# brucechin/OctopusZK

Hardware: AMD Instinct MI355X
Metric: BN254 G1 VariableBaseMSM Mscalar-mul/s at 2^20 (higher is better)
Workload: dtype u32; 1 GPU; VariableBaseMSM BN254 G1 2^20 random scalars/bases per GPU, bit-exact vs the serial CPU path (BASELINE.json configs[1]); n_per_gpu=1048576, window_bits=16, windows=8, glv=True, prepared_bases=False, msms_in_flight=3, schedule=pipeline3, parallelism=index-range shard x1, RCCL all-gather of 192-B partials + HIP point sum

## Files before the change

### include/ozk.h

```cpp
#ifndef OZK_H
#define OZK_H

#include <stddef.h>
#include <stdint.h>

#ifdef __cplusplus
extern "C" {
#endif

#define OZK_OK 0
#define OZK_E_INVALID -1
#define OZK_E_NO_DEVICE -2
#define OZK_E_NOMEM -3
#define OZK_E_INTERNAL -4

#define OZK_G1 1
#define OZK_G2 2

const char* ozk_last_error(void);
int ozk_version(void);
int ozk_device_count(void);
int ozk_device_cu_count(void);
int ozk_stream_create_cu_range(int32_t first_cu, int32_t n_cus, void** stream);
int ozk_stream_destroy(void* stream);
// ... 32 lines not shown
int ozk_var_msm_stage_bytes(int32_t n, int32_t type, size_t* sorted_bytes, size_t* sort_ws_bytes,
                            size_t* accum_ws_bytes);
int ozk_var_msm_sort_dev(const void* d_bases, int32_t prepared, const void* d_scalars, int32_t n, int32_t type,
                         void* d_sorted, size_t sorted_bytes, void* d_sort_ws, size_t sort_ws_bytes, void* stream);
int ozk_var_msm_accum_dev(const void* d_prepared, int32_t n, int32_t type, void* d_sorted, size_t sorted_bytes,
                          void* d_accum_ws, size_t accum_ws_bytes, void* d_tail, size_t tail_bytes, void* stream,
                          int32_t part);

size_t ozk_var_msm_prepared_bytes(int32_t n, int32_t type);
int ozk_var_msm_prepare_dev(const void* d_bases, int32_t n, int32_t type, void* d_prepared, size_t prepared_size,
                            void* stream);
int ozk_var_msm_prepared_dev(const void* d_prepared, const void* d_scalars, int32_t n, int32_t type, void* d_out,
                             void* d_workspace, size_t workspace_bytes, void* stream);
int ozk_bases_create_host(const uint8_t* bases, int32_t n, int32_t type, int32_t task_id, void** handle);
int ozk_var_msm_bases_host(void* handle, const uint8_t* scalars, int32_t n, uint8_t* out);
int ozk_bases_destroy(void* handle);
int ozk_bases_type(void* handle);

int ozk_order_event_create(void** ev);
int ozk_order_event_destroy(void* ev);


int ozk_points_sum_dev(const void* d_points, int32_t k, int32_t type, void* d_out, void* stream);

int ozk_groth16_combine_dev(const void* d_records, int32_t world, void* d_proof, void* stream);

int ozk_prof_enable(int on);
int ozk_prof_dominant_kernel_ms(double* avg_ms, int* launches);
int ozk_prof_dominant_kernel_stats(double* stats4, int* launches);
int ozk_prof_dominant_kernel_clock_mhz(double* stats4, int* launches);
double ozk_prof_clock_khz(void);
int ozk_var_msm_plan(int32_t n, int32_t* window_bits, int32_t* windows);
int ozk_var_msm_glv(int32_t n);

int ozk_gen_bases_dev(uint64_t seed, int32_t n, int32_t type, void* d_out_wire, void* stream);

int ozk_fixed_batch_msm_host(int32_t outerc, int32_t window_size, int32_t out_len,
                             int32_t inner_len, int32_t n, int32_t scalar_size,
                             const uint8_t* base, const uint8_t* scalars, int32_t bn_type,
                             int32_t task_id, uint8_t* out);
int ozk_fixed_double_batch_msm_host(int32_t outerc1, int32_t window_size1, int32_t outerc2,
                                    int32_t window_size2, int32_t out_len1, int32_t inner_len1,
                                    int32_t out_len2, int32_t inner_len2, int32_t n,
                                    const uint8_t* base_g1, const uint8_t* base_g2,
                                    const uint8_t* scalars, int32_t task_id, uint8_t* out);
int ozk_field_batch_mul_host(const uint8_t* in, int32_t n, int32_t task_id, uint8_t* out);

size_t ozk_fixed_batch_msm_workspace_bytes(int32_t outerc, int32_t window_size, int32_t n,
                                           int32_t bn_type);
int ozk_fixed_batch_msm_dev(int32_t outerc, int32_t window_size, int32_t n, const void* d_base,
                            const void* d_scalars, int32_t bn_type, void* d_out,
                            void* d_workspace, size_t workspace_bytes, void* stream);
int ozk_field_batch_mul_dev(const void* d_in, int32_t n, void* d_out, void* stream);
int ozk_fixed_batch_msm_compact_dev(int32_t outerc, int32_t window_size, int32_t n, const void* d_base,
                                    const void* d_scalars, int32_t bn_type, void* d_out, void* d_workspace,
                                    size_t workspace_bytes, void* stream);
int ozk_fixed_batch_msm_compact_host(int32_t outerc, int32_t window_size, int32_t n, const uint8_t* base,
                                     const uint8_t* scalars, int32_t bn_type, int32_t task_id, uint8_t* out);
int ozk_fixed_batch_msm_base_dev(int32_t outerc, int32_t window_size, int32_t n, const uint8_t* base_host,
                                 const void* d_scalars, int32_t bn_type, void* d_out, int32_t compact,
                                 void* d_workspace, size_t workspace_bytes, void* stream);

int ozk_fft_host(const uint8_t* in, int32_t n, const uint8_t* omega, int32_t task_id,
                 uint8_t* out);
size_t ozk_fft_workspace_bytes(int32_t n);
int ozk_fft_dev(const void* d_in, int32_t n, const uint8_t* omega_host32, void* d_out,
// ... 94 lines not shown
```

### octopuszk_amd/build.py

```python
import os
import shutil
import subprocess
import sys

HERE = os.path.dirname(os.path.abspath(__file__))
CSRC = os.path.join(HERE, "csrc")
ROOT = os.path.dirname(HERE)
LIB = os.path.join(HERE, "libozk_hip.so")

HIP_SOURCES = ["msm_var.hip", "msm_var_g2.hip", "msm_fixed.hip", "fft.hip", "host_ctx.hip", "pairing.hip", "msm_multi.hip",
               "point_codec.hip", "points_scale.hip", "ec_fft.hip"]
HEADERS = ["consts_gen.h", "mad_chain_gen.h", "fp29.cuh", "fq2.cuh", "fq12.cuh", "batch_verify.cuh", "point_codec.cuh", "points_scale.cuh", "ec_fft.cuh", "bace.cuh", "pairing_consts_gen.h", "ec.cuh", "quad.cuh", "curve.cuh", "msm_var.cuh", "msm_var_driver.cuh", "msm_multi.cuh", "glv.cuh", "ozk_common.h", "knobs.h", "host_ctx.h", "pin_cache.h",
           os.path.join("..", "..", "include", "ozk.h")]
HIPCC_FLAGS = ["-std=c++17", "-O3", "--offload-arch=gfx950", "-fPIC", "-fno-gpu-rdc", "-Wno-unused-result",
               "-Wno-pass-failed"]

JNI_LIBS = {
    "libAlgebraMSMVariableBaseMSM.so": "jni_var_msm.c",
    "libAlgebraMSMFixedBaseMSM.so": "jni_fixed_msm.c",
    "libAlgebraFFTAuxiliary.so": "jni_fft.c",
}


def _newer(target, deps):
    if not os.path.exists(target):
        return True
    t = os.path.getmtime(target)
    return any(os.path.exists(d) and os.path.getmtime(d) > t for d in deps)


def hipcc():
    for cand in (shutil.which("hipcc"), "/opt/rocm/bin/hipcc"):
        if cand and os.path.exists(cand):
            return cand
    raise RuntimeError("hipcc not found: the HIP library cannot be built (there is no CPU path)")


def build(force=False, verbose=True):
    srcs = [os.path.join(CSRC, s) for s in HIP_SOURCES if os.path.exists(os.path.join(CSRC, s))]
    deps = srcs + [os.path.join(CSRC, h) for h in HEADERS]
    if force or _newer(LIB, deps):
        defs = []
        if os.path.exists(os.path.join(CSRC, "fq2.cuh")):
            defs.append("-DOZK_WITH_G2")
        objdir = os.path.join(HERE, "_obj")
# ... 38 lines not shown
```

### octopuszk_amd/csrc/knobs.h

```cpp
#pragma once
#include <stdlib.h>
#include <string.h>

#include <atomic>
#include <mutex>

namespace ozk {

constexpr int KNOB_COMPUTED = -0x7fffffff;
constexpr int KNOB_STRING = KNOB_COMPUTED + 1;

#define OZK_KNOBS(X)                                                                                                     \
                                                   \
  X(MSM_GLV, "OZK_MSM_GLV", 1, "0: plain 256-bit windows instead of the GLV split (var MSM up to 2^23 pairs, fixed base)") \
  X(MSM_SIGNED, "OZK_MSM_SIGNED", 1, "0: unsigned window digits in the GLV form")                                        \
  X(MSM_C, "OZK_MSM_C", KNOB_COMPUTED, "window bits, 1..16 (default: the cost model's choice)")                          \
  X(MSM_L1, "OZK_MSM_L1", KNOB_COMPUTED, "sorted entries per level-1 lane (default: from the bucket size; 0 as unset)")   \
  X(MSM_L1_ROUNDS, "OZK_MSM_L1_ROUNDS", 2, "most rounds of resident workgroups level 1 is rounded up to; 0: no rounding") \
  X(MSM_TAIL_MODE, "OZK_MSM_TAIL_MODE", -1, "0 / 1: force the latency / throughput shape of the window sums")            \
  X(MSM_SMALL_SORT, "OZK_MSM_SMALL_SORT", 1, "0: small MSMs take the two-level sort too")                                \
  X(MSM_S_LAT, "OZK_MSM_S_LAT", KNOB_COMPUTED, "buckets per lane in a latency tail's fused first level (default: 8 G1, 4 G2)") \
  X(MSM_FIN_MAX, "OZK_MSM_FIN_MAX", 4, "elements per window left to the final one-wave kernel, 1..16")                   \
                                                                                                    \
  X(HOST_SLICES, "OZK_HOST_SLICES", 8, "most slices a host-buffer MSM is cut into; 1: no slicing")                       \
  X(HOST_SLICE_MIN_LOG, "OZK_HOST_SLICE_MIN_LOG", 18, "log2 of the smallest slice")                                      \
  X(SHARD, "OZK_SHARD", 0, "1: the JNI entries shard large calls over the visible devices")                              \
  X(SHARD_MIN_N, "OZK_SHARD_MIN_N", 1 << 21, "smallest call OZK_SHARD=1 shards")                                         \
  X(SHARD_COUNT, "OZK_SHARD_COUNT", 0, "shards of such a call; 0: one per device")                                       \
  X(SHARD_RCCL, "OZK_SHARD_RCCL", 1, "0: the partials of a sharded call go through the host, not RCCL")                  \
  X(COPY_HELPERS, "OZK_COPY_HELPERS", 3, "threads staging host buffers beside the caller, 0..11 (first use only)")       \
  X(HOST_TRACE, "OZK_HOST_TRACE", 0, "1: per-call host timings on stderr; 2: with absolute timestamps")                  \
                                                                                     \
  X(FB_WS, "OZK_FB_WS", KNOB_COMPUTED, "window bits of a GLV fixed-base table (default: cost model, at most the caller's)") \
  X(FB_AFFINE, "OZK_FB_AFFINE", 1, "0: Jacobian gather-add instead of affine table records")                             \
  X(FB_TABLE_CACHE, "OZK_FB_TABLE_CACHE", 1, "0: window tables are built per call")                                      \
  X(FB_TABLE_CACHE_MB, "OZK_FB_TABLE_CACHE_MB", 1024, "MiB of cached window tables per device")                          \
  X(FB_TABLE_CACHE_SECOND_USE, "OZK_FB_TABLE_CACHE_SECOND_USE", 1, "0: a table is cached on its first use")              \
  X(FB_HOST_RANGES, "OZK_FB_HOST_RANGES", 4, "ranges a host fixed-base call downloads its results in")                   \
  X(MM_WS, "OZK_MM_WS", KNOB_COMPUTED, "window bits of the shared-base batched MSM (default: from n)")                   \
                                                                                             \
  X(FFT_MAXK, "OZK_FFT_MAXK", 8, "most butterfly stages per pass, 3..10")                                                \
  X(FFT_PLAN, "OZK_FFT_PLAN", 1, "0: stages spread evenly over the passes")                                              \
  X(FFT_KS, "OZK_FFT_KS", KNOB_STRING, "explicit stages per pass, e.g. \"8,6,8\" (must sum to log2 n)")                  \
  X(FFT_TW_PYRAMID, "OZK_FFT_TW_PYRAMID", 1, "0: twiddles from the flat table")                                          \
  X(FFT_PLAN_CACHE, "OZK_FFT_PLAN_CACHE", 1, "0: twiddle tables are built per call")                                     \
  X(FFT_PLAN_CACHE_MB, "OZK_FFT_PLAN_CACHE_MB", 4096, "MiB of cached twiddle tables per device")                         \
  X(QAP_FOLD_SCALE, "OZK_QAP_FOLD_SCALE", 1, "0: the witness map scales in a pass of its own")                           \
  X(BACE_LDS_SLOTS, "OZK_BACE_LDS_SLOTS", 16, "circuit slots kept in LDS, 0..28")

enum Knob {
// ... 58 lines not shown
```

### octopuszk_amd/csrc/msm_var.cuh

```cuda
#pragma once
#include "curve.cuh"
#include "glv.cuh"

namespace ozk {

constexpr u32 BID_NONE = 0xffffffffu;

struct MsmPlan {
  int n_in;
  int glv;
  int n;
  int sd;
  int c;
  int cb;
  int W;
  int L1;
  int LK;
  int S;
  int lone;
  int small_sort;
  int S_lat;
  int fin_max;
  int tail_mode;
};

OZK_HD u32 scalar_digit(const u32 (&s)[8], int w, int c) {
  const int bit = w * c;
  const int wi = bit >> 5, sh = bit & 31;
  u32 v = s[wi] >> sh;
  if (sh + c > 32 && wi + 1 < 8) v |= s[wi + 1] << (32 - sh);
  return v & ((1u << c) - 1u);
}

OZK_HD bool digit_decode(u32 code, int sd, u32& b, u32& neg) {
  if (sd) {
    const u32 t = code - 1u;
    b = t >> 1;
    neg = t & 1u;
  } else {
    b = code;
    neg = 0;
  }
  return code != 0;
}
template <class Emit>
OZK_HD void signed_digit_codes(const u32 (&e)[8], int c, int W, bool neg, Emit emit) {
  const u32 half = 1u << (c - 1);
  const u32 thr = (c == 16 && neg) ? half - 1u : half;
  u32 cy = 0;
  for (int w = 0; w < W; w++) {
    const u32 d = scalar_digit(e, w, c) + cy;
    cy = d > thr;
    const u32 m = cy ? (1u << c) - d : d;
    emit(w, (uint16_t)(m ? (((m - 1u) << 1) | (cy ^ (u32)neg)) + 1u : 0u));
  }
}
// ... 907 lines not shown
        acc.accumulate(pts_in, idx_in, p);
      }
    }
    }
    if (cur != BID_NONE) {
      if (cur_cb) {
        head_bid = cur;
        acc.store(pts_out + (size_t)(2 * (size_t)t) * IO::REC_WORDS);
        if (cf) {
          tail_bid = cur;
          if constexpr (FIRST) {
            acc.store_infinity(pts_out + (size_t)(2 * (size_t)t + 1) * IO::REC_WORDS);
          } else {
            IO::store_rec_jac(jac_infinity<CV>(), pts_out + (size_t)(2 * (size_t)t + 1) * IO::REC_WORDS);
          }
        }
      } else if (cf) {
        tail_bid = cur;
        acc.store(pts_out + (size_t)(2 * (size_t)t + 1) * IO::REC_WORDS);
      } else {
        acc.store(buckets + (size_t)cur * IO::REC_WORDS);
      }
    }
  }
  bid_out[2 * (size_t)t] = head_bid;
  bid_out[2 * (size_t)t + 1] = tail_bid;
}

template <class CV, bool FIRST, bool LAZY = false>
__global__ void __launch_bounds__(256, (FIRST && CV::LDS_ACC) ? 2 : 1)
k_segreduce(const u32* __restrict__ bid_in, const u32* __restrict__ idx_in, const u32* __restrict__ pts_in,
            const u32* __restrict__ d_count, int n_in_static, int L,
            u32* __restrict__ buckets, u32* __restrict__ bid_out, u32* __restrict__ pts_out,
            int n_lanes, unsigned long long* __restrict__ clk) {
  const int t = blockIdx.x * blockDim.x + threadIdx.x;
  unsigned long long w0 = 0, c0 = 0;
  if constexpr (FIRST) {
    if (clk != nullptr && threadIdx.x == 0) {
      w0 = (unsigned long long)wall_clock64();
      c0 = (unsigned long long)clock64();
      atomicMax(&clk[0], ~w0);
    }
  }
  if (t < n_lanes)
    segreduce_lane<CV, FIRST, LAZY>(t, bid_in, idx_in, pts_in, d_count, n_in_static, L, buckets, bid_out, pts_out);
  if constexpr (FIRST) {
    if (clk != nullptr && (threadIdx.x & 63) == 0) {
      const unsigned long long w1 = (unsigned long long)wall_clock64();
      atomicMax(&clk[1], w1);
      if (threadIdx.x == 0) {
        atomicAdd(&clk[2], (unsigned long long)clock64() - c0);
        atomicAdd(&clk[3], w1 - w0);
      }
    }
  }
}

static __global__ void k_read_clock(unsigned long long* out) { out[0] = (unsigned long long)wall_clock64(); }

template <class CV>
__global__ void __launch_bounds__(256)
k_segreduce_small(const u32* __restrict__ d_count, int n_in, int L, u32* __restrict__ buckets,
                  u32* __restrict__ bid_a, u32* __restrict__ pts_a, u32* __restrict__ bid_b, u32* __restrict__ pts_b) {
  if (*d_count == 0) return;
  u32 *bi = bid_a, *pi = pts_a, *bo = bid_b, *po = pts_b;
  while (true) {
    const int lanes = (n_in + L - 1) / L;
    for (int t = threadIdx.x; t < lanes; t += blockDim.x)
      segreduce_lane<CV, false>(t, bi, nullptr, pi, d_count, n_in, L, buckets, bo, po);
    if (lanes == 1) break;
    block_sync();
    n_in = 2 * lanes;
    u32* tb = bi; bi = bo; bo = tb;
    u32* tp = pi; pi = po; po = tp;
  }
}

constexpr int RUN_MAX = 16;
constexpr int RUNMERGE_BLOCK = 256;
template <class CV>
__global__ void __launch_bounds__(RUNMERGE_BLOCK)
k_runmerge(const u32* __restrict__ bid_in, const u32* __restrict__ pts, int n_slots,
           u32* __restrict__ buckets, u32* __restrict__ bid_out, u32* __restrict__ remaining,
           const u32* __restrict__ hist_src, u32* __restrict__ hist_dst, size_t n_hist) {
  using IO = CurveIO<CV>;
  constexpr bool LIST = !CV::LDS_ACC;
  constexpr int ROUNDS = RUN_MAX / 2;
  constexpr int CAP = 2 * RUNMERGE_BLOCK;
  __shared__ u32 item_s[2][CAP];
  __shared__ uint8_t item_span[2][CAP];
  __shared__ u32 item_cnt[ROUNDS + 1];
  if (threadIdx.x <= ROUNDS) item_cnt[threadIdx.x] = 0;
  const int t = blockIdx.x * blockDim.x + threadIdx.x;
  for (size_t i = (size_t)t; i < n_hist; i += (size_t)gridDim.x * blockDim.x) hist_dst[i] = hist_src[i];
  block_sync();
  u32 alive = 0;
#pragma unroll 1
  for (int k = 0; k < 2; k++) {
    const int x = 2 * t + 1 + k;
    if (x >= n_slots) break;
    const u32 bx = bid_in[x];
    u32 out = BID_NONE;
    if (bx != BID_NONE) {
      int s = x, e = x;
      while (s > 0 && x - s < RUN_MAX && bid_in[s - 1] == bx) s--;
      while (e + 1 < n_slots && e - x < RUN_MAX && bid_in[e + 1] == bx) e++;
      const bool is_short = (x - s < RUN_MAX) && (e - x < RUN_MAX) && (e - s + 1 <= RUN_MAX);
      if (!is_short) {
        out = bx;
      } else if (s == x) {
        if constexpr (!LIST) {
          Xyzz<CV> acc = IO::load_xyzz(pts + (size_t)s * IO::REC_WORDS);
          for (int q = s + 1; q <= e; q += 2) acc = xyzz_add(acc, IO::load_xyzz(pts + (size_t)q * IO::REC_WORDS));
          IO::store_rec_xyzz(acc, buckets + (size_t)bx * IO::REC_WORDS);
        } else if (e > s) {
          const u32 j = atomicAdd(&item_cnt[0], 1u);
          item_s[0][j] = (u32)s;
          item_span[0][j] = (uint8_t)(e - s);
        } else {
          IO::store_rec_xyzz(IO::load_xyzz(pts + (size_t)s * IO::REC_WORDS), buckets + (size_t)bx * IO::REC_WORDS);
        }
      }
    }
    bid_out[x] = out;
    alive += (out != BID_NONE);
  }
  if (t == 0 && n_slots > 0) {
    bid_out[0] = bid_in[0];
    alive += (bid_in[0] != BID_NONE);
  }
  for (int o = 32; o > 0; o >>= 1) alive += __shfl_xor(alive, o);
  if ((threadIdx.x & 63) == 0 && alive) atomicAdd(remaining, alive);
#pragma unroll 1
  for (int r = 0; LIST && r < ROUNDS; r++) {
    block_sync();
    const u32 len = (u32)__builtin_amdgcn_readfirstlane((int)item_cnt[r]);
    if (len == 0) break;
    const int cur = r & 1;
#pragma unroll 1
    for (u32 i = threadIdx.x; i < len; i += RUNMERGE_BLOCK) {
      const u32 s = item_s[cur][i];
      const u32 span = item_span[cur][i];
      u32* bucket = buckets + (size_t)bid_in[s] * IO::REC_WORDS;
      const u32 off = 2u * (u32)r + 1u;
      const u32* sum = r == 0 ? pts + (size_t)s * IO::REC_WORDS : bucket;
      const Xyzz<CV> acc = xyzz_add(IO::load_xyzz(sum), IO::load_xyzz(pts + ((size_t)s + off) * IO::REC_WORDS));
      IO::store_rec_xyzz(acc, bucket);
      if (off + 2u <= span) {
        const u32 j = atomicAdd(&item_cnt[r + 1], 1u);
        item_s[cur ^ 1][j] = s;
        item_span[cur ^ 1][j] = (uint8_t)span;
      }
    }
  }
}

template <class CV, bool FIRSTLEVEL>
__global__ void __launch_bounds__(256)
k_wsum(const u32* __restrict__ A_in, const u32* __restrict__ R_in, const u32* __restrict__ hist,
       int m_in, int S, int g, u32* __restrict__ A_out, u32* __restrict__ R_out, int m_out, int W, int prio) {
  using IO = CurveIO<CV>;
  if (prio) __builtin_amdgcn_s_setprio(3);
  const int t = blockIdx.x * blockDim.x + threadIdx.x;
  if (t >= m_out * W) return;
  const int w = t / m_out, j = t - w * m_out;
  const size_t base = (size_t)w * m_in;
  const int lo = j * S;
  int hi = lo + S;
  if (hi > m_in) hi = m_in;
  Jac<CV> run = jac_infinity<CV>(), ws = jac_infinity<CV>(), asum = jac_infinity<CV>();
  for (int e = hi - 1; e >= lo; e--) {
    if constexpr (FIRSTLEVEL) {
      if (hist[base + e] != 0) run = jac_add(run, IO::load_rec(R_in + (base + e) * IO::REC_WORDS));
    } else {
      run = jac_add(run, IO::load_jac(R_in + (base + e) * IO::JAC_WORDS));
    }
    if (e > lo) ws = jac_add(ws, run);
    if constexpr (!FIRSTLEVEL) asum = jac_add(asum, IO::load_jac(A_in + (base + e) * IO::JAC_WORDS));
  }
  for (int k = 0; k < g; k++) ws = jac_dbl(ws);
  if constexpr (!FIRSTLEVEL) ws = jac_add(ws, asum);
  IO::store_jac(ws, A_out + ((size_t)w * m_out + j) * IO::JAC_WORDS);
  IO::store_jac(run, R_out + ((size_t)w * m_out + j) * IO::JAC_WORDS);
}

// ... 254 lines not shown
```

### octopuszk_amd/csrc/msm_var.hip

```cpp
#include "msm_var_driver.cuh"

#include <dlfcn.h>
#include <rccl/rccl.h>

#include <algorithm>
#include <chrono>
#include <new>
#include <string>
#include <thread>
#include <vector>

OZK_G2_DRIVER_INSTANCES(extern)

using namespace ozk;

template <class F>
static auto with_plan(int n, int type, F f) {
  return by_point_type(type, [&](auto t) { return f(t, plan_for<typename decltype(t)::CV>(n, false)); });
}
#define CV_OF(t) typename decltype(t)::CV

extern "C" {

size_t ozk_var_msm_workspace_bytes(int32_t n, int32_t type) {
// ... 732 lines not shown
  OZK_HIP(hipDeviceSynchronize());
  std::vector<unsigned long long> h((size_t)g_prof.count * 4);
  if (g_prof.count) OZK_HIP(hipMemcpy(h.data(), g_prof.d_clk, h.size() * sizeof(unsigned long long), hipMemcpyDeviceToHost));
  std::vector<double> m;
  double tot = 0;
  for (int i = 0; i < g_prof.count; i++) {
    if (h[4 * i + 3] == 0) continue;
    const double mhz = (double)h[4 * i + 2] / (double)h[4 * i + 3] * g_prof.clk_khz * 1e-3;
    m.push_back(mhz);
    tot += mhz;
  }
  *launches = (int)m.size();
  if (m.empty()) return OZK_OK;
  std::sort(m.begin(), m.end());
  stats4[0] = tot / (double)m.size();
  stats4[1] = m[m.size() / 2];
  stats4[2] = m.front();
  stats4[3] = m.back();
  return OZK_OK;
}

double ozk_prof_clock_khz(void) { return g_prof.clk_khz; }

int ozk_var_msm_plan(int32_t n, int32_t* window_bits, int32_t* windows) {
  if (n <= 0 || !window_bits || !windows) return fail(OZK_E_INVALID, "bad argument");
  const MsmPlan p = make_plan(n);
  *window_bits = p.c;
  *windows = p.W;
  return OZK_OK;
}

int ozk_var_msm_glv(int32_t n) { return n > 0 ? make_plan(n).glv : 0; }

const char* ozk_last_error(void) { return err_buf(); }
int ozk_version(void) { return 2; }
int ozk_device_count(void) {
  int n = 0;
  if (hipGetDeviceCount(&n) != hipSuccess) return 0;
  return n;
}

}
```

### octopuszk_amd/csrc/msm_var_driver.cuh

```cuda
#pragma once
#include <hip/hip_ext.h>
#include <pthread.h>
#include <stdlib.h>

#include <atomic>
#include <vector>

#include "msm_var.cuh"
#include "host_ctx.h"
#include "fq2.cuh"

namespace ozk {

enum { PROF_OFF = 0, PROF_EVENTS = 1, PROF_CLOCK = 2 };
struct ProfState {
  pthread_mutex_t mu = PTHREAD_MUTEX_INITIALIZER;
  std::atomic<int> mode{PROF_OFF};
  int src = PROF_EVENTS;
  int every = 1, seen = 0;
  int count = 0;
  std::vector<hipEvent_t> e0, e1;
  bool created = false;
  int ev_device = -1;
  unsigned long long* d_clk = nullptr;
// ... 73 lines not shown
  p.sd = sd_ok && c >= 2;
  p.cb = c - p.sd;
  p.W = ((p.glv ? 128 : 256) + c - 1) / c;
  {
    const long long per_bucket = (long long)p.n >> p.cb;
    long long l1 = per_bucket * 5 / 16;
    long long l1_min = p.n >= (1 << 20) ? 52 : 40;
    if (p.glv) {
      const long long cap = (long long)p.n * p.W;
      long long fit = cap / 65536;
      const int top_bits = 127 - (p.W - 1) * p.c;
      const int tb = top_bits - p.sd;
      const long long per_top = (top_bits >= 1 && top_bits < p.c) ? ((long long)p.n >> (tb > 0 ? tb : 0)) : per_bucket;
      const long long pieces = (per_top + 9) / 10;
      if (fit < pieces) fit = pieces;
      if (fit < 8) fit = 8;
      if (fit < l1_min) l1_min = fit;
    }
    if (l1 < l1_min) l1 = l1_min;
    if (l1 > 1024) l1 = 1024;
    p.L1 = knob_or(K_MSM_L1, (int)l1);
  }
  if (p.L1 < 2) p.L1 = 2;
  p.LK = PLAN_LK;
  p.S = PLAN_S;
  p.lone = 0;
  p.small_sort = p.n <= SORTS_MAX_N && p.cb <= SORTS_MAX_CB && knob(K_MSM_SMALL_SORT) != 0;
  p.S_lat = p.S;
  p.fin_max = knob(K_MSM_FIN_MAX);
  if (p.fin_max < 1) p.fin_max = 1;
  if (p.fin_max > 16) p.fin_max = 16;
  p.tail_mode = knob(K_MSM_TAIL_MODE);
  if (p.tail_mode != 0 && p.tail_mode != 1) p.tail_mode = -1;
  return p;
}

template <class CV>
static MsmPlan plan_for(int n, bool lone) {
  MsmPlan p = make_plan(n);
  p.lone = lone;
  const long long max_rounds = knob(K_MSM_L1_ROUNDS);
  if ((CV::LDS_ACC || lone) && knob_or(K_MSM_L1, 0) == 0 && max_rounds != 0) {
    static int cu_count = 0;
    if (cu_count == 0) {
      int dev = 0, cus = 0;
      if (hipGetDevice(&dev) == hipSuccess && hipDeviceGetAttribute(&cus, hipDeviceAttributeMultiprocessorCount, dev) == hipSuccess &&
          cus > 0)
        cu_count = cus;
      else
        cu_count = 256;
    }
    const int slots = (CV::LDS_ACC ? 2 : 3) * cu_count;
    const long long cap = (long long)p.n * p.W;
    const long long blocks = ((cap + p.L1 - 1) / p.L1 + 255) / 256;
    long long rounds = blocks / slots > 0 ? blocks / slots : 1;
    if (rounds > max_rounds) rounds = max_rounds;
    long long l1 = (cap + 256LL * slots * rounds - 1) / (256LL * slots * rounds);
    if (l1 > p.L1 && l1 <= 1024) p.L1 = (int)l1;
  }
  const int s_lat = knob_or(K_MSM_S_LAT, std::is_same<CV, G1Cfg>::value && p.cb >= 13 ? 8 : p.S);
  if (s_lat >= 2 && s_lat <= 64) p.S_lat = 1 << ilog2((uint32_t)s_lat);
  return p;
}

struct MsmLayout {
  u32* aff;
  u32 *hist, *C1, *P1, *blocksum, *total;
  uint16_t* digits;
  uint8_t* neg_flags;
  u32* coarse;
  uint2* sent;
  BigBins* bigbins;
  u32* bigT;
  size_t big_items_max;
  int lo_bits, NH, nblk;
  size_t nC1;
  u32* buckets;
  u32* hist_t;
  u32 *slot_bid[2], *slot_pts[2], *slot_bid2;
  u32 *wA[2], *wR[2];
  size_t bytes;
  size_t cap;
  size_t NB;
  size_t slots0, slots1;
  size_t m1;
};

struct RegionBytes {
  size_t sorted, sort_ws, accum_ws;
};
template <class CV>
MsmLayout make_layout3(const MsmPlan& p, void* sorted, void* sort_ws, void* accum_ws, RegionBytes* rb,
                              const void* prepared = nullptr) {
  using IO = CurveIO<CV>;
  MsmLayout L;
  L.cap = (size_t)p.n * p.W;
// ... 144 lines not shown
  const u32 big_thresh = (u32)(n / 64) > SORT_BIG ? (u32)(n / 64) : SORT_BIG;
  if (L.cap / ((size_t)big_thresh + 1) > (size_t)SORTBIG_MAXBINS)
    return fail(OZK_E_INVALID, "window plan c=%d (W=%d) at n=%d can produce more than %d oversized sort bins",
                p.c, p.W, p.n_in, SORTBIG_MAXBINS);
  hipLaunchKernelGGL(k_sort2, dim3(nbins), dim3(SORT2_BLOCK), 0, st, L.coarse, L.P1, L.total, p.cb, L.lo_bits, L.NH,
                     sign_bit, L.nblk, nbins, big_thresh, L.hist, L.sent);
  if (order_ev) OZK_HIP(hipStreamWaitEvent(st, order_ev, 0));
  hipLaunchKernelGGL(k_sortbig_list, dim3(1), dim3(256), 0, st, L.P1, L.total, L.nblk, nbins, big_thresh, L.bigbins);
  hipLaunchKernelGGL(k_sortbig_count, dim3(1024), dim3(SORT_BLOCK), 0, st, L.coarse, L.bigbins,
                     (1u << L.lo_bits) - 1u, L.bigT);
  hipLaunchKernelGGL(k_sortbig_scan, dim3(SORTBIG_MAXBINS), dim3(256), 0, st, L.bigbins, L.bigT, p.cb, L.lo_bits, L.NH,
                     L.hist);
  hipLaunchKernelGGL(k_sortbig_scatter, dim3(1024), dim3(SORT_BLOCK), 0, st, L.coarse, L.bigbins, L.bigT, p.cb,
                     L.lo_bits, sign_bit, L.NH, L.sent);
  OZK_HIP(hipGetLastError());
  return OZK_OK;
}

enum { ACCUM_ALL = 0, ACCUM_LEVEL1 = 1, ACCUM_REST = 2 };
template <class CV>
int var_msm_accum(const MsmPlan& p, void* sorted, size_t sorted_bytes, void* accum_ws, size_t accum_ws_bytes,
                         void* tail, size_t tail_bytes, hipStream_t st, const void* prepared = nullptr,
                         int part = ACCUM_ALL) {
  hip_clear_stale();
  using CT = CV;
  RegionBytes rb;
  MsmLayout L = make_layout3<CV>(p, sorted, nullptr, accum_ws, &rb, prepared);
  if (rb.sorted > sorted_bytes || rb.accum_ws > accum_ws_bytes)
    return fail(OZK_E_INVALID, "accumulate buffers too small: need %zu + %zu bytes, got %zu + %zu", rb.sorted,
                rb.accum_ws, sorted_bytes, accum_ws_bytes);
  const size_t tneed = tail_layout<CV>(p, L, tail, tail_bytes);
  if (tneed > tail_bytes) return fail(OZK_E_INVALID, "tail buffer too small: need %zu bytes, got %zu", tneed, tail_bytes);
  const int TB = 256;
  size_t lanes = (L.cap + p.L1 - 1) / p.L1;
  if (part != ACCUM_REST) {
  hipEvent_t prof_e0 = nullptr, prof_e1 = nullptr;
  unsigned long long* clk = nullptr;
  g_prof.claim(&prof_e0, &prof_e1, &clk);
  const bool prof = prof_e0 != nullptr;
  size_t acc_lds = CV::LDS_ACC ? (size_t)RunAccLds<CV>::LDS_WORDS * TB * sizeof(u32) : 0;
  if (!CV::LDS_ACC) acc_lds = L1_LDS_G1;
  auto launch_l1 = [&](auto kern) {
    if (acc_lds > 65536)
      OZK_HIP(hipFuncSetAttribute((const void*)kern, hipFuncAttributeMaxDynamicSharedMemorySize, (int)acc_lds));
    hipExtLaunchKernelGGL(kern, dim3((unsigned)((lanes + TB - 1) / TB)), dim3(TB), (uint32_t)acc_lds, st,
                          prof ? prof_e0 : (hipEvent_t) nullptr, prof ? prof_e1 : (hipEvent_t) nullptr, 0u,
                          (const u32*)nullptr, (const u32*)L.sent, (const u32*)L.aff, (const u32*)L.total, 0, p.L1,
                          L.buckets, L.slot_bid[0], L.slot_pts[0], (int)lanes, clk);
    return OZK_OK;
  };
  if (int rc_l1 = launch_l1(k_segreduce<CV, true, CV::LAZY_MADD>)) return rc_l1;
  }
  if (part == ACCUM_LEVEL1) {
    OZK_HIP(hipGetLastError());
    return OZK_OK;
  }
  size_t n_in = 2 * lanes;
  static_assert(RUNMERGE_BLOCK == 256, "k_runmerge's work list is sized for this launch");
  hipLaunchKernelGGL((k_runmerge<CT>), dim3((unsigned)((lanes + TB - 1) / TB)), dim3(TB), 0, st, L.slot_bid[0],
                     L.slot_pts[0], (int)n_in, L.buckets, L.slot_bid2, L.total + 1, (const u32*)L.hist, L.hist_t, L.NB);
  int cur = 0;
  bool first_generic = true;
  while (true) {
    lanes = (n_in + p.LK - 1) / p.LK;
    if (!first_generic && (int)lanes <= SMALL_LEVEL_LANES) {
      hipLaunchKernelGGL((k_segreduce_small<CT>), dim3(1), dim3(TB), 0, st, L.total + 1, (int)n_in, p.LK, L.buckets,
                         L.slot_bid[cur], L.slot_pts[cur], L.slot_bid[cur ^ 1], L.slot_pts[cur ^ 1]);
      break;
    }
    hipLaunchKernelGGL((k_segreduce<CT, false>), dim3((unsigned)((lanes + TB - 1) / TB)), dim3(TB), 0, st,
                       first_generic ? L.slot_bid2 : L.slot_bid[cur], (const u32*)nullptr, L.slot_pts[cur],
                       L.total + 1, (int)n_in, p.LK, L.buckets, L.slot_bid[cur ^ 1], L.slot_pts[cur ^ 1], (int)lanes,
                       (unsigned long long*)nullptr);
    first_generic = false;
    if (lanes == 1) break;
    n_in = 2 * lanes;
    cur ^= 1;
  }
  OZK_HIP(hipGetLastError());
  return OZK_OK;
}

template <class CV>
int var_msm_head(const MsmPlan& p, const void* d_bases, const void* d_scalars, void* ws, size_t ws_bytes, void* tail,
                        size_t tail_bytes, hipStream_t st, hipEvent_t order_ev = nullptr,
                        const void* prepared = nullptr) {
  const RegionBytes rb = region_bytes<CV>(p);
  if (rb.sorted + rb.sort_ws + rb.accum_ws > ws_bytes)
    return fail(OZK_E_INVALID, "workspace too small: need %zu bytes, got %zu", rb.sorted + rb.sort_ws + rb.accum_ws,
                ws_bytes);
  uint8_t* w = (uint8_t*)ws;
  int rc = var_msm_sort<CV>(p, d_bases, d_scalars, w, rb.sorted, w + rb.sorted, rb.sort_ws, st, order_ev, prepared);
  if (rc) return rc;
// ... 318 lines not shown
```

### octopuszk_amd/lib.py

```python
import ctypes
import os

HERE = os.path.dirname(os.path.abspath(__file__))
LIB_PATH = os.environ.get("OZK_LIB_PATH") or os.path.join(HERE, "libozk_hip.so")

_lib = None

c_u8p = ctypes.POINTER(ctypes.c_uint8)
i32 = ctypes.c_int32
vp = ctypes.c_void_p
sz = ctypes.c_size_t

_SIGS = {
    "ozk_last_error": (ctypes.c_char_p, []),
    "ozk_version": (ctypes.c_int, []),
    "ozk_device_count": (ctypes.c_int, []),
    "ozk_var_msm_host": (ctypes.c_int, [vp, vp, i32, i32, i32, vp]),
    "ozk_var_double_msm_host": (ctypes.c_int, [vp, vp, vp, i32, i32, vp]),
    "ozk_var_msm_sharded_host": (ctypes.c_int, [vp, vp, i32, i32, i32, vp]),
    "ozk_var_msm_auto_host": (ctypes.c_int, [vp, vp, i32, i32, i32, vp]),
    "ozk_var_double_msm_sharded_host": (ctypes.c_int, [vp, vp, vp, i32, i32, vp]),
    "ozk_var_double_msm_auto_host": (ctypes.c_int, [vp, vp, vp, i32, i32, vp]),
    "ozk_shard_last_exchange": (ctypes.c_int, []),
    "ozk_shard_comms_release": (None, []),
    "ozk_var_msm_workspace_bytes": (sz, [i32, i32]),
    "ozk_var_msm_dev": (ctypes.c_int, [vp, vp, i32, i32, vp, vp, sz, vp]),
    "ozk_prof_enable": (ctypes.c_int, [ctypes.c_int]),
    "ozk_prof_dominant_kernel_ms": (ctypes.c_int, [ctypes.POINTER(ctypes.c_double), ctypes.POINTER(ctypes.c_int)]),
    "ozk_prof_dominant_kernel_stats": (ctypes.c_int, [ctypes.POINTER(ctypes.c_double), ctypes.POINTER(ctypes.c_int)]),
    "ozk_prof_clock_khz": (ctypes.c_double, []),
    "ozk_prof_dominant_kernel_clock_mhz": (ctypes.c_int, [ctypes.POINTER(ctypes.c_double), ctypes.POINTER(ctypes.c_int)]),
    "ozk_var_msm_plan": (ctypes.c_int, [i32, ctypes.POINTER(i32), ctypes.POINTER(i32)]),
    "ozk_var_msm_glv": (ctypes.c_int, [i32]),
    "ozk_gen_bases_dev": (ctypes.c_int, [ctypes.c_uint64, i32, i32, vp, vp]),
    "ozk_var_msm_stage_bytes": (ctypes.c_int, [i32, i32, ctypes.POINTER(sz), ctypes.POINTER(sz), ctypes.POINTER(sz)]),
    "ozk_var_msm_sort_dev": (ctypes.c_int, [vp, i32, vp, i32, i32, vp, sz, vp, sz, vp]),
    "ozk_var_msm_accum_dev": (ctypes.c_int, [vp, i32, i32, vp, sz, vp, sz, vp, sz, vp, i32]),
    "ozk_device_cu_count": (ctypes.c_int, []),
    "ozk_stream_create_cu_range": (ctypes.c_int, [i32, i32, ctypes.POINTER(ctypes.c_void_p)]),
    "ozk_stream_destroy": (ctypes.c_int, [vp]),
    "ozk_var_msm_head_workspace_bytes": (sz, [i32, i32]),
    "ozk_var_msm_tail_bytes": (sz, [i32, i32]),
    "ozk_var_msm_head_dev": (ctypes.c_int, [vp, i32, vp, i32, i32, vp, sz, vp, sz, vp, vp]),
    "ozk_var_msm_tail_dev": (ctypes.c_int, [i32, i32, vp, sz, vp, vp, vp, i32]),
    "ozk_bases_create_host": (ctypes.c_int, [vp, i32, i32, i32, ctypes.POINTER(vp)]),
    "ozk_var_msm_bases_host": (ctypes.c_int, [vp, vp, i32, vp]),
    "ozk_bases_destroy": (ctypes.c_int, [vp]),
    "ozk_var_msm_prepared_bytes": (sz, [i32, i32]),
    "ozk_var_msm_prepare_dev": (ctypes.c_int, [vp, i32, i32, vp, sz, vp]),
    "ozk_var_msm_prepared_dev": (ctypes.c_int, [vp, vp, i32, i32, vp, vp, sz, vp]),
    "ozk_order_event_create": (ctypes.c_int, [ctypes.POINTER(vp)]),
    "ozk_order_event_destroy": (ctypes.c_int, [vp]),
    "ozk_points_sum_dev": (ctypes.c_int, [vp, i32, i32, vp, vp]),
    "ozk_groth16_combine_dev": (ctypes.c_int, [vp, i32, vp, vp]),
    "ozk_fixed_batch_msm_host": (ctypes.c_int, [i32, i32, i32, i32, i32, i32, vp, vp, i32, i32, vp]),
    "ozk_fixed_double_batch_msm_host": (ctypes.c_int, [i32] * 9 + [vp, vp, vp, i32, vp]),
    "ozk_field_batch_mul_host": (ctypes.c_int, [vp, i32, i32, vp]),
    "ozk_fixed_batch_msm_workspace_bytes": (sz, [i32, i32, i32, i32]),
    "ozk_fixed_batch_msm_dev": (ctypes.c_int, [i32, i32, i32, vp, vp, i32, vp, vp, sz, vp]),
    "ozk_field_batch_mul_dev": (ctypes.c_int, [vp, i32, vp, vp]),
    "ozk_fixed_batch_msm_compact_dev": (ctypes.c_int, [i32, i32, i32, vp, vp, i32, vp, vp, sz, vp]),
    "ozk_fixed_batch_msm_compact_host": (ctypes.c_int, [i32, i32, i32, vp, vp, i32, i32, vp]),
    "ozk_fixed_batch_msm_base_dev": (ctypes.c_int, [i32, i32, i32, vp, vp, i32, vp, i32, vp, sz, vp]),
    "ozk_fft_compact_host": (ctypes.c_int, [vp, i32, vp, i32, vp]),
    "ozk_fft_compact_dev": (ctypes.c_int, [vp, i32, vp, vp, vp, sz, vp]),
    "ozk_tuning_reload": (ctypes.c_int, []),
# ... 88 lines not shown
```

Baseline: 729.2 Mscalar-mul/s.

## Add whole-bucket level-1 accumulation path on lane groups for G1 GLV MSM

Adds a level-1 bucket accumulation path that gives each whole bucket to a group of two or four lanes, ordered by rank of bucket size, and combines the partial sums with DPP quad swaps. This removes the segmented-reduce and run-merge passes when every bucket fits. Two small kernels build per-bin prefix sums and bucket items, and they set a device-side 'bad' flag that sends the work back to the old segreduce and runmerge kernels when buckets are too large. The knob defaults to 1, so the new path is enabled on every G1 GLV signed plan that qualifies. The cost is extra launches, a guard check in the old kernels, and possible lane imbalance from skewed buckets.

```diff
diff --git a/include/ozk.h b/include/ozk.h
--- a/include/ozk.h
+++ b/include/ozk.h
@@ -88,6 +88,7 @@
 double ozk_prof_clock_khz(void);
 int ozk_var_msm_plan(int32_t n, int32_t* window_bits, int32_t* windows);
 int ozk_var_msm_glv(int32_t n);
+int ozk_var_msm_last_l1_path(void);
 
 int ozk_gen_bases_dev(uint64_t seed, int32_t n, int32_t type, void* d_out_wire, void* stream);
 
diff --git a/octopuszk_amd/build.py b/octopuszk_amd/build.py
--- a/octopuszk_amd/build.py
+++ b/octopuszk_amd/build.py
@@ -10,7 +10,7 @@
 
 HIP_SOURCES = ["msm_var.hip", "msm_var_g2.hip", "msm_fixed.hip", "fft.hip", "host_ctx.hip", "pairing.hip", "msm_multi.hip",
                "point_codec.hip", "points_scale.hip", "ec_fft.hip"]
-HEADERS = ["consts_gen.h", "mad_chain_gen.h", "fp29.cuh", "fq2.cuh", "fq12.cuh", "batch_verify.cuh", "point_codec.cuh", "points_scale.cuh", "ec_fft.cuh", "bace.cuh", "pairing_consts_gen.h", "ec.cuh", "quad.cuh", "curve.cuh", "msm_var.cuh", "msm_var_driver.cuh", "msm_multi.cuh", "glv.cuh", "ozk_common.h", "knobs.h", "host_ctx.h", "pin_cache.h",
+HEADERS = ["consts_gen.h", "mad_chain_gen.h", "fp29.cuh", "fq2.cuh", "fq12.cuh", "batch_verify.cuh", "point_codec.cuh", "points_scale.cuh", "ec_fft.cuh", "bace.cuh", "pairing_consts_gen.h", "ec.cuh", "quad.cuh", "curve.cuh", "msm_var.cuh", "msm_var_driver.cuh", "msm_multi.cuh", "glv.cuh", "l1_whole.h", "ozk_common.h", "knobs.h", "host_ctx.h", "pin_cache.h",
            os.path.join("..", "..", "include", "ozk.h")]
 HIPCC_FLAGS = ["-std=c++17", "-O3", "--offload-arch=gfx950", "-fPIC", "-fno-gpu-rdc", "-Wno-unused-result",
                "-Wno-pass-failed"]
diff --git a/octopuszk_amd/csrc/knobs.h b/octopuszk_amd/csrc/knobs.h
--- a/octopuszk_amd/csrc/knobs.h
+++ b/octopuszk_amd/csrc/knobs.h
@@ -16,6 +16,7 @@
   X(MSM_SIGNED, "OZK_MSM_SIGNED", 1, "0: unsigned window digits in the GLV form")                                        \
   X(MSM_C, "OZK_MSM_C", KNOB_COMPUTED, "window bits, 1..16 (default: the cost model's choice)")                          \
   X(MSM_L1, "OZK_MSM_L1", KNOB_COMPUTED, "sorted entries per level-1 lane (default: from the bucket size; 0 as unset)")   \
+  X(MSM_L1_WHOLE, "OZK_MSM_L1_WHOLE", 1, "G1 level 1 by whole buckets on lane groups: 0 never, 1 on every plan that can take it (unset: where it pays)") \
   X(MSM_L1_ROUNDS, "OZK_MSM_L1_ROUNDS", 2, "most rounds of resident workgroups level 1 is rounded up to; 0: no rounding") \
   X(MSM_TAIL_MODE, "OZK_MSM_TAIL_MODE", -1, "0 / 1: force the latency / throughput shape of the window sums")            \
   X(MSM_SMALL_SORT, "OZK_MSM_SMALL_SORT", 1, "0: small MSMs take the two-level sort too")                                \
diff --git a/octopuszk_amd/csrc/l1_whole.h b/octopuszk_amd/csrc/l1_whole.h
--- /dev/null
+++ b/octopuszk_amd/csrc/l1_whole.h
@@ -0,0 +1,71 @@
+#pragma once
+#include <stdint.h>
+
+#if !defined(OZK_HD)
+#if defined(__HIPCC__)
+#include <hip/hip_runtime.h>
+#define OZK_HD __host__ __device__ __forceinline__
+#else
+#define OZK_HD inline
+#endif
+#endif
+
+namespace ozk {
+
+constexpr int WHOLE_G = 2;
+constexpr int WHOLE_LANE_MAX = 255;
+constexpr int WHOLE_NB_MAX = 128;
+
+struct WholeGeom {
+  int W;
+  int NH;
+  int nb;
+  int g_top;
+};
+OZK_HD int whole_nbins(const WholeGeom& g) { return g.W * g.NH; }
+constexpr uint32_t WHOLE_NO_ITEM = 0xffffffffu;
+OZK_HD int whole_pad4(int x) { return (x + 3) & ~3; }
+OZK_HD int whole_lanes_per_rank(const WholeGeom& g) {
+  return whole_pad4(WHOLE_G * g.NH * (g.W - 1)) + whole_pad4(g.g_top * g.NH);
+}
+OZK_HD long long whole_lanes(const WholeGeom& g) { return (long long)g.nb * whole_lanes_per_rank(g); }
+OZK_HD int whole_group(const WholeGeom& g, int bin) { return bin / g.NH == g.W - 1 ? g.g_top : WHOLE_G; }
+OZK_HD uint32_t whole_limit(int G) { return (uint32_t)(G * WHOLE_LANE_MAX); }
+
+OZK_HD uint32_t whole_rank(const uint32_t* cnt, int nb, int i) {
+  const uint32_t c = cnt[i];
+  uint32_t r = 0;
+  for (int j = 0; j < nb; j++) r += (cnt[j] > c) || (cnt[j] == c && j < i);
+  return r;
+}
+OZK_HD uint32_t whole_item_index(uint32_t rank, uint32_t bin, uint32_t nbins) { return rank * nbins + bin; }
+
+OZK_HD void whole_lane_map(const WholeGeom& geo, uint32_t t, uint32_t* item, uint32_t* g, uint32_t* G) {
+  const uint32_t per_rank = (uint32_t)whole_lanes_per_rank(geo);
+  const uint32_t rank = t / per_rank, q = t - rank * per_rank;
+  const uint32_t ordinary = (uint32_t)(WHOLE_G * geo.NH * (geo.W - 1));
+  const uint32_t ordinary_pad = (uint32_t)whole_pad4((int)ordinary);
+  uint32_t bin;
+  bool pad;
+  if (q < ordinary_pad) {
+    bin = q / WHOLE_G;
+    *g = q % WHOLE_G;
+    *G = WHOLE_G;
+    pad = q >= ordinary;
+  } else {
+    const uint32_t q2 = q - ordinary_pad;
+    bin = (uint32_t)(geo.NH * (geo.W - 1)) + q2 / (uint32_t)geo.g_top;
+    *g = q2 % (uint32_t)geo.g_top;
+    *G = (uint32_t)geo.g_top;
+    pad = q2 >= (uint32_t)(geo.g_top * geo.NH);
+  }
+  *item = pad ? WHOLE_NO_ITEM : whole_item_index(rank, bin, (uint32_t)whole_nbins(geo));
+}
+
+OZK_HD void whole_part(uint32_t count, uint32_t g, uint32_t G, uint32_t* first, uint32_t* len) {
+  const uint32_t a = (count * g + G - 1) / G, b = (count * (g + 1) + G - 1) / G;
+  *first = a;
+  *len = b - a;
+}
+
+}
diff --git a/octopuszk_amd/csrc/msm_var.cuh b/octopuszk_amd/csrc/msm_var.cuh
--- a/octopuszk_amd/csrc/msm_var.cuh
+++ b/octopuszk_amd/csrc/msm_var.cuh
@@ -1,6 +1,7 @@
 #pragma once
 #include "curve.cuh"
 #include "glv.cuh"
+#include "l1_whole.h"
 
 namespace ozk {
 
@@ -22,6 +23,8 @@
   int S_lat;
   int fin_max;
   int tail_mode;
+  int l1_whole;
+  int l1_gtop;
 };
 
 OZK_HD u32 scalar_digit(const u32 (&s)[8], int w, int c) {
@@ -995,7 +998,10 @@
 k_segreduce(const u32* __restrict__ bid_in, const u32* __restrict__ idx_in, const u32* __restrict__ pts_in,
             const u32* __restrict__ d_count, int n_in_static, int L,
             u32* __restrict__ buckets, u32* __restrict__ bid_out, u32* __restrict__ pts_out,
-            int n_lanes, unsigned long long* __restrict__ clk) {
+            int n_lanes, unsigned long long* __restrict__ clk, const u32* __restrict__ whole_bad = nullptr) {
+  if constexpr (FIRST) {
+    if (whole_bad != nullptr && *whole_bad == 0) return;
+  }
   const int t = blockIdx.x * blockDim.x + threadIdx.x;
   unsigned long long w0 = 0, c0 = 0;
   if constexpr (FIRST) {
@@ -1045,7 +1051,8 @@
 __global__ void __launch_bounds__(RUNMERGE_BLOCK)
 k_runmerge(const u32* __restrict__ bid_in, const u32* __restrict__ pts, int n_slots,
            u32* __restrict__ buckets, u32* __restrict__ bid_out, u32* __restrict__ remaining,
-           const u32* __restrict__ hist_src, u32* __restrict__ hist_dst, size_t n_hist) {
+           const u32* __restrict__ hist_src, u32* __restrict__ hist_dst, size_t n_hist,
+           const u32* __restrict__ whole_bad = nullptr) {
   using IO = CurveIO<CV>;
   constexpr bool LIST = !CV::LDS_ACC;
   constexpr int ROUNDS = RUN_MAX / 2;
@@ -1056,6 +1063,7 @@
   if (threadIdx.x <= ROUNDS) item_cnt[threadIdx.x] = 0;
   const int t = blockIdx.x * blockDim.x + threadIdx.x;
   for (size_t i = (size_t)t; i < n_hist; i += (size_t)gridDim.x * blockDim.x) hist_dst[i] = hist_src[i];
+  if (whole_bad != nullptr && *whole_bad == 0) return;
   block_sync();
   u32 alive = 0;
 #pragma unroll 1
@@ -1114,6 +1122,126 @@
         item_s[cur ^ 1][j] = s;
         item_span[cur ^ 1][j] = (uint8_t)span;
       }
+    }
+  }
+}
+
+constexpr int ITEMS_BLOCK = WHOLE_NB_MAX;
+__device__ __forceinline__ u32 items_block_sum(u32 v, u32* wsum) {
+#pragma unroll
+  for (int o = 32; o > 0; o >>= 1) v += __shfl_xor(v, o);
+  if ((threadIdx.x & 63) == 0) wsum[threadIdx.x >> 6] = v;
+  block_sync();
+  return wsum[0] + wsum[1];
+}
+static __global__ void __launch_bounds__(ITEMS_BLOCK)
+k_bin_sums(const u32* __restrict__ hist, WholeGeom geo, int cb, int lo_bits, u32* __restrict__ binsum) {
+  static_assert(ITEMS_BLOCK == 128, "two waves");
+  __shared__ u32 wsum[2];
+  const int t = threadIdx.x, bin = blockIdx.x;
+  const int w = bin / geo.NH, h = bin - w * geo.NH;
+  const u32 bucket0 = ((u32)w << cb) | ((u32)h << lo_bits);
+  const u32 sum = items_block_sum(t < geo.nb ? hist[bucket0 + t] : 0u, wsum);
+  if (t == 0) binsum[bin] = sum;
+}
+static __global__ void __launch_bounds__(ITEMS_BLOCK)
+k_bucket_items(const u32* __restrict__ hist, const u32* __restrict__ binsum, WholeGeom geo, int cb, int lo_bits,
+               u32 big_thresh, uint4* __restrict__ items, u32* __restrict__ bad) {
+  __shared__ u32 cnt[WHOLE_NB_MAX];
+  __shared__ u32 wsum[2];
+  const int t = threadIdx.x, bin = blockIdx.x;
+  const int w = bin / geo.NH, h = bin - w * geo.NH;
+  const u32 bucket0 = ((u32)w << cb) | ((u32)h << lo_bits);
+  const u32 c = t < geo.nb ? hist[bucket0 + t] : 0u;
+  cnt[t] = c;
+  u32 before = 0;
+  for (int j = t; j < bin; j += ITEMS_BLOCK) before += binsum[j];
+  const u32 base = items_block_sum(before, wsum);
+  if (t >= geo.nb) return;
+  u32 excl = 0, sum = 0;
+  for (int j = 0; j < geo.nb; j++) {
+    const u32 cj = cnt[j];
+    sum += cj;
+    excl += j < t ? cj : 0u;
+  }
+  const u32 rank = whole_rank(cnt, geo.nb, t);
+  items[whole_item_index(rank, (u32)bin, (u32)whole_nbins(geo))] = make_uint4(base + excl, c, bucket0 + (u32)t, 0u);
+  if (c > whole_limit(whole_group(geo, bin)) || sum > big_thresh) *bad = 1u;
+}
+
+template <int CTRL, class CV>
+__device__ __forceinline__ Xyzz<CV> xyzz_quad_swap(const Xyzz<CV>& a) {
+  using IO = CurveIO<CV>;
+  constexpr int RW = IO::RW;
+  u32 w[4 * RW];
+  ElemTraits<typename CV::XX>::store_raw(a.X, w);
+  ElemTraits<typename CV::XY>::store_raw(a.Y, w + RW);
+  ElemTraits<typename CV::XZZ>::store_raw(a.ZZ, w + 2 * RW);
+  ElemTraits<typename CV::XZZZ>::store_raw(a.ZZZ, w + 3 * RW);
+#pragma unroll
+  for (int k = 0; k < 4 * RW; k++) w[k] = (u32)__builtin_amdgcn_update_dpp(0, (int)w[k], CTRL, 0xf, 0xf, true);
+  Xyzz<CV> b;
+  b.X = ElemTraits<typename CV::XX>::load_raw(w);
+  b.Y = ElemTraits<typename CV::XY>::load_raw(w + RW);
+  b.ZZ = ElemTraits<typename CV::XZZ>::load_raw(w + 2 * RW);
+  b.ZZZ = ElemTraits<typename CV::XZZZ>::load_raw(w + 3 * RW);
+  return b;
+}
+
+template <class CV>
+__global__ void __launch_bounds__(256)
+k_l1_whole(const uint4* __restrict__ items, const uint2* __restrict__ sent, const u32* __restrict__ pts_in,
+           const u32* __restrict__ bad, WholeGeom geo, u32 n_lanes, u32* __restrict__ buckets,
+           unsigned long long* __restrict__ clk) {
+  using IO = CurveIO<CV>;
+  using Acc = RunAcc<CV, true>;
+  if (*bad != 0u) return;
+  unsigned long long w0 = 0, c0 = 0;
+  if (clk != nullptr && threadIdx.x == 0) {
+    w0 = (unsigned long long)wall_clock64();
+    c0 = (unsigned long long)clock64();
+    atomicMax(&clk[0], ~w0);
+  }
+  const u32 t = blockIdx.x * blockDim.x + threadIdx.x;
+  u32 item, g, G;
+  whole_lane_map(geo, t < n_lanes ? t : 0u, &item, &g, &G);
+  const bool valid = t < n_lanes && item != WHOLE_NO_ITEM;
+  uint4 it = items[valid ? item : 0u];
+  if (!valid) it.y = 0u;
+  u32 first, n_e;
+  whole_part(it.y, g, G, &first, &n_e);
+  Xyzz<CV> a = xyzz_from_affine<CV>(IO::aff_infinity());
+  if (n_e != 0u) {
+    const u32* idx_c = reinterpret_cast<const u32*>(sent + (size_t)it.x + first);
+    u32 v_cur = idx_c[0];
+    u32 v_next = idx_c[n_e > 1u ? 2 : 0];
+    const __amdgpu_buffer_rsrc_t table = Acc::table_rsrc(pts_in);
+    typename Acc::Raw r = Acc::load_raw_buf(table, v_cur);
+    for (u32 k = 0; k < n_e; k++) {
+      const bool negate = (v_cur & SIDX_NEG) != 0;
+      const auto q = Acc::decode_unsigned(r);
+      const u32 k2 = (k + 2 < n_e) ? k + 2 : n_e - 1;
+      r = Acc::load_raw_buf(table, v_next);
+      v_cur = v_next;
+      v_next = idx_c[2 * (size_t)k2];
+      a = xyzz_madd_lazy(a, q, negate);
+    }
+  }
+  if (__ballot(G > 1u) != 0ull) {
+    const Xyzz<CV> b = xyzz_quad_swap<0xB1, CV>(a);
+    if (G > 1u) a = xyzz_add(a, b);
+  }
+  if (__ballot(G > 2u) != 0ull) {
+    const Xyzz<CV> b = xyzz_quad_swap<0x4E, CV>(a);
+    if (G > 2u) a = xyzz_add(a, b);
+  }
+  if (g == 0u && it.y != 0u) IO::store_rec_xyzz(a, buckets + (size_t)it.z * IO::REC_WORDS);
+  if (clk != nullptr && (threadIdx.x & 63) == 0) {
+    const unsigned long long w1 = (unsigned long long)wall_clock64();
+    atomicMax(&clk[1], w1);
+    if (threadIdx.x == 0) {
+      atomicAdd(&clk[2], (unsigned long long)clock64() - c0);
+      atomicAdd(&clk[3], w1 - w0);
     }
   }
 }
diff --git a/octopuszk_amd/csrc/msm_var.hip b/octopuszk_amd/csrc/msm_var.hip
--- a/octopuszk_amd/csrc/msm_var.hip
+++ b/octopuszk_amd/csrc/msm_var.hip
@@ -788,6 +788,17 @@
 
 int ozk_var_msm_glv(int32_t n) { return n > 0 ? make_plan(n).glv : 0; }
 
+int ozk_var_msm_last_l1_path(void) {
+  const L1PathLast& last = g_l1_path_last;
+  if (last.planned <= 0) return last.planned;
+  u32 bad = 0;
+  if (hipDeviceSynchronize() != hipSuccess || hipMemcpy(&bad, last.d_bad, sizeof(bad), hipMemcpyDeviceToHost) != hipSuccess) {
+    (void)hipGetLastError();
+    return -1;
+  }
+  return bad ? 0 : 1;
+}
+
 const char* ozk_last_error(void) { return err_buf(); }
 int ozk_version(void) { return 2; }
 int ozk_device_count(void) {
diff --git a/octopuszk_amd/csrc/msm_var_driver.cuh b/octopuszk_amd/csrc/msm_var_driver.cuh
--- a/octopuszk_amd/csrc/msm_var_driver.cuh
+++ b/octopuszk_amd/csrc/msm_var_driver.cuh
@@ -129,6 +129,8 @@
   if (p.fin_max > 16) p.fin_max = 16;
   p.tail_mode = knob(K_MSM_TAIL_MODE);
   if (p.tail_mode != 0 && p.tail_mode != 1) p.tail_mode = -1;
+  p.l1_whole = 0;
+  p.l1_gtop = WHOLE_G;
   return p;
 }
 
@@ -137,6 +139,7 @@
   MsmPlan p = make_plan(n);
   p.lone = lone;
   const long long max_rounds = knob(K_MSM_L1_ROUNDS);
+  bool rounded = false;
   if ((CV::LDS_ACC || lone) && knob_or(K_MSM_L1, 0) == 0 && max_rounds != 0) {
     static int cu_count = 0;
     if (cu_count == 0) {
@@ -153,12 +156,34 @@
     long long rounds = blocks / slots > 0 ? blocks / slots : 1;
     if (rounds > max_rounds) rounds = max_rounds;
     long long l1 = (cap + 256LL * slots * rounds - 1) / (256LL * slots * rounds);
-    if (l1 > p.L1 && l1 <= 1024) p.L1 = (int)l1;
+    if (l1 > p.L1 && l1 <= 1024) {
+      p.L1 = (int)l1;
+      rounded = true;
+    }
   }
   const int s_lat = knob_or(K_MSM_S_LAT, std::is_same<CV, G1Cfg>::value && p.cb >= 13 ? 8 : p.S);
   if (s_lat >= 2 && s_lat <= 64) p.S_lat = 1 << ilog2((uint32_t)s_lat);
+  const int whole_knob = knob_or(K_MSM_L1_WHOLE, -1);
+  bool whole_pays = true;
+  if (lone) {
+    const int tb = 127 - (p.W - 1) * p.c;
+    const long long per_bucket = (long long)p.n >> p.cb;
+    const long long per_top = (tb >= 1 && tb < p.c) ? ((long long)p.n >> (tb - p.sd > 0 ? tb - p.sd : 0)) : per_bucket;
+    whole_pays = !rounded && per_bucket / WHOLE_G <= p.L1 && per_top / 4 <= p.L1;
+  }
+  if (std::is_same<CV, G1Cfg>::value && p.glv && p.sd && !p.small_sort && (whole_knob == -1 ? whole_pays : whole_knob != 0)) {
+    const int top_bits = 127 - (p.W - 1) * p.c;
+    p.l1_whole = 1;
+    p.l1_gtop = (top_bits >= 1 && top_bits < p.c) ? 4 : WHOLE_G;
+  }
   return p;
 }
+
+struct L1PathLast {
+  int planned = -1;
+  const u32* d_bad = nullptr;
+};
+inline thread_local L1PathLast g_l1_path_last;
 
 struct MsmLayout {
   u32* aff;
@@ -369,6 +394,11 @@
   const size_t tneed = tail_layout<CV>(p, L, tail, tail_bytes);
   if (tneed > tail_bytes) return fail(OZK_E_INVALID, "tail buffer too small: need %zu bytes, got %zu", tneed, tail_bytes);
   const int TB = 256;
+  const bool whole = !CV::LDS_ACC && p.l1_whole && (1 << L.lo_bits) <= WHOLE_NB_MAX &&
+                     L.NB * sizeof(uint4) + (size_t)p.W * L.NH * sizeof(u32) <= rb.accum_ws;
+  u32* whole_bad = L.total + 2;
+  g_l1_path_last.planned = whole ? 1 : 0;
+  g_l1_path_last.d_bad = whole_bad;
   size_t lanes = (L.cap + p.L1 - 1) / p.L1;
   if (part != ACCUM_REST) {
   hipEvent_t prof_e0 = nullptr, prof_e1 = nullptr;
@@ -381,11 +411,28 @@
     if (acc_lds > 65536)
       OZK_HIP(hipFuncSetAttribute((const void*)kern, hipFuncAttributeMaxDynamicSharedMemorySize, (int)acc_lds));
     hipExtLaunchKernelGGL(kern, dim3((unsigned)((lanes + TB - 1) / TB)), dim3(TB), (uint32_t)acc_lds, st,
-                          prof ? prof_e0 : (hipEvent_t) nullptr, prof ? prof_e1 : (hipEvent_t) nullptr, 0u,
+                          prof && !whole ? prof_e0 : (hipEvent_t) nullptr, prof && !whole ? prof_e1 : (hipEvent_t) nullptr, 0u,
                           (const u32*)nullptr, (const u32*)L.sent, (const u32*)L.aff, (const u32*)L.total, 0, p.L1,
-                          L.buckets, L.slot_bid[0], L.slot_pts[0], (int)lanes, clk);
+                          L.buckets, L.slot_bid[0], L.slot_pts[0], (int)lanes, clk, whole ? (const u32*)whole_bad : (const u32*)nullptr);
     return OZK_OK;
   };
+  if constexpr (!CV::LDS_ACC) {
+    if (whole) {
+      const WholeGeom geo{p.W, L.NH, 1 << L.lo_bits, p.l1_gtop};
+      const u32 big_thresh = (u32)(p.n / 64) > SORT_BIG ? (u32)(p.n / 64) : SORT_BIG;
+      uint4* items = (uint4*)accum_ws;
+      u32* binsum = (u32*)(items + L.NB);
+      hipLaunchKernelGGL(k_bin_sums, dim3((unsigned)whole_nbins(geo)), dim3(ITEMS_BLOCK), 0, st, (const u32*)L.hist, geo,
+                         p.cb, L.lo_bits, binsum);
+      hipLaunchKernelGGL(k_bucket_items, dim3((unsigned)whole_nbins(geo)), dim3(ITEMS_BLOCK), 0, st, (const u32*)L.hist,
+                         (const u32*)binsum, geo, p.cb, L.lo_bits, big_thresh, items, whole_bad);
+      const long long wl = whole_lanes(geo);
+      hipExtLaunchKernelGGL((k_l1_whole<CV>), dim3((unsigned)((wl + TB - 1) / TB)), dim3(TB), (uint32_t)acc_lds, st,
+                            prof ? prof_e0 : (hipEvent_t) nullptr, prof ? prof_e1 : (hipEvent_t) nullptr, 0u,
+                            (const uint4*)items, (const uint2*)L.sent, (const u32*)L.aff, (const u32*)whole_bad, geo,
+                            (u32)wl, L.buckets, clk);
+    }
+  }
   if (int rc_l1 = launch_l1(k_segreduce<CV, true, CV::LAZY_MADD>)) return rc_l1;
   }
   if (part == ACCUM_LEVEL1) {
@@ -395,7 +442,8 @@
   size_t n_in = 2 * lanes;
   static_assert(RUNMERGE_BLOCK == 256, "k_runmerge's work list is sized for this launch");
   hipLaunchKernelGGL((k_runmerge<CT>), dim3((unsigned)((lanes + TB - 1) / TB)), dim3(TB), 0, st, L.slot_bid[0],
-                     L.slot_pts[0], (int)n_in, L.buckets, L.slot_bid2, L.total + 1, (const u32*)L.hist, L.hist_t, L.NB);
+                     L.slot_pts[0], (int)n_in, L.buckets, L.slot_bid2, L.total + 1, (const u32*)L.hist, L.hist_t, L.NB,
+                     whole ? (const u32*)whole_bad : (const u32*)nullptr);
   int cur = 0;
   bool first_generic = true;
   while (true) {
diff --git a/octopuszk_amd/lib.py b/octopuszk_amd/lib.py
--- a/octopuszk_amd/lib.py
+++ b/octopuszk_amd/lib.py
@@ -32,6 +32,7 @@
     "ozk_prof_dominant_kernel_clock_mhz": (ctypes.c_int, [ctypes.POINTER(ctypes.c_double), ctypes.POINTER(ctypes.c_int)]),
     "ozk_var_msm_plan": (ctypes.c_int, [i32, ctypes.POINTER(i32), ctypes.POINTER(i32)]),
     "ozk_var_msm_glv": (ctypes.c_int, [i32]),
+    "ozk_var_msm_last_l1_path": (ctypes.c_int, []),
     "ozk_gen_bases_dev": (ctypes.c_int, [ctypes.c_uint64, i32, i32, vp, vp]),
     "ozk_var_msm_stage_bytes": (ctypes.c_int, [i32, i32, ctypes.POINTER(sz), ctypes.POINTER(sz), ctypes.POINTER(sz)]),
     "ozk_var_msm_sort_dev": (ctypes.c_int, [vp, i32, vp, i32, i32, vp, sz, vp, sz, vp]),
```

Measured after the change: 741.7 Mscalar-mul/s, median of 6. 1.7% higher.
